# YuvalBahat/Explorable-Super-Resolution

Hardware: AMD Instinct MI355X
Metric: HR pixels/sec (RRDB-23 x4, 128->512, bs32 per GPU, fwd + CEM) (higher is better)
Workload: dtype bf16x3 (bf16 hi+lo operands = 16 significand bits per operand in every product, three MFMAs, f32 accumulate)

## Files before the change

### explorable-super-resolution_amd/csrc/esr_conv.hip

```cpp
#include "esr_common.h"
#include <type_traits>
#include <vector>

namespace {

constexpr int NW = 4;
constexpr int NTHREADS = 64 * NW;
constexpr int MAXS_BASE = 3;
constexpr int WGS_MT1 = 2, WGS_MT2 = 2;
constexpr int r_of(int mt) { return 3; }
constexpr int maxs_of(int mt) { return r_of(mt) > 3 ? MAXS_BASE + 1 : MAXS_BASE; }

typedef __attribute__((ext_vector_type(4))) unsigned int u32x4;
constexpr int EPI_RES1 = 1, EPI_RES2 = 2, EPI_MASK = 4, EPI_NCHW = 8, EPI_OUT2 = 16;
constexpr int EPI_RESIN = 32;
constexpr int EPI_PS = 64;

struct ConvArgs {
    int tiles_x, tiles_y, ntiles;
    int xcd_q, xcd_r;
    unsigned m_tx, m_ty;
    unsigned i_tx, i_ty;
    int TH, TW, P, NPIX_T, NPIX_L, nslots;
    unsigned m_P, m_ups;
    int H, W, Win_p, ups;
    unsigned share[NW];
    int ncp, lo_chunks, reverse, B;
    DView in0, in1;
    const uint4* wpack;
    long long wchunk;
    long long wslice;
    int wtap;
    int nslices;
    const float* zero_bias;
    int bias_stride;
    const float* bias;
    int cout, ncg_out;
    float act_slope, alpha, beta1, beta2;
    DView res1, res2, out, out2, mask;
    float* out_nchw;
    int mask_cg0, mask_cg1;
    float mask_slope;
    int resin_g0;
    float resin_scale;
    int ps, ps_rg0;
    unsigned m_ns, i_ns;
    int ph_off;
    int ksplit, kz_groups;
    long long kz_slab;
    int nchw_ctot;
    int stages_hint;
    unsigned* range_flag;
    unsigned range_tag;
#ifdef ESR_TRACE
    unsigned long long* trace;
#endif
};

typedef __attribute__((ext_vector_type(8))) _Float16 f16x8;
typedef __attribute__((ext_vector_type(2))) float f32x2;
template <int FMT>
__device__ __forceinline__ f32x16 mfma(uint4 a, uint4 b, f32x16 c) {
    if (FMT) return __builtin_amdgcn_mfma_f32_32x32x16_f16(__builtin_bit_cast(f16x8, a), __builtin_bit_cast(f16x8, b), c, 0, 0, 0);
    return __builtin_amdgcn_mfma_f32_32x32x16_bf16(__builtin_bit_cast(bf16x8, a), __builtin_bit_cast(bf16x8, b), c, 0, 0, 0);
}
template <int FMT>
__device__ __forceinline__ uint32_t cvt_pk(float lo, float hi);

__device__ __forceinline__ uint32_t cvt_pk_bf16(float lo, float hi) {
    uint32_t r;
    asm("v_cvt_pk_bf16_f32 %0, %1, %2" : "=v"(r) : "v"(lo), "v"(hi));
    return r;
}
template <> __device__ __forceinline__ uint32_t cvt_pk<0>(float lo, float hi) { return cvt_pk_bf16(lo, hi); }
template <> __device__ __forceinline__ uint32_t cvt_pk<1>(float lo, float hi) { return f2h(lo) | (f2h(hi) << 16); }

__device__ __forceinline__ void glds16s(const uint4* sbase, unsigned voff, unsigned lds_dst) {
    asm volatile("s_mov_b32 m0, %2\n\ts_nop 0\n\tglobal_load_lds_dwordx4 %0, %1" : : "v"(voff), "s"(sbase), "s"(__builtin_amdgcn_readfirstlane(lds_dst)) : "memory");
}

__device__ __forceinline__ unsigned udiv_magic(unsigned n, unsigned m, unsigned i) { return __umulhi(n, m) + n * i; }

__device__ __forceinline__ const uint4* in_plane(const ConvArgs& a, int g, int b, bool lo) {
    if (g < a.in0.ncg) return (lo ? a.in0.lo : a.in0.hi) + b * a.in0.bs + g * a.in0.cs;
    int g1 = g - a.in0.ncg;
    if (g1 >= a.in1.ncg) g1 = 0;
    return (lo ? a.in1.lo : a.in1.hi) + b * a.in1.bs + g1 * a.in1.cs;
}

template <int MAXS>
struct FetchState {
    unsigned soff[MAXS];
    int slot[MAXS];
};

template <int MAXS>
__device__ __forceinline__ FetchState<MAXS> setup_tile(const ConvArgs& a, int x0, int y0, int wave, int lane) {
    FetchState<MAXS> f;
#pragma unroll
    for (int s = 0; s < MAXS; ++s) {
        f.slot[s] = (wave + s * NW) < a.nslots ? wave + s * NW : wave;
        const unsigned p = (unsigned)f.slot[s] * 64 + lane;
        const unsigned rr = __umul24(p, a.m_P) >> 20, cc = p - rr * a.P;
        const unsigned Yp = y0 + rr, Xp = x0 + cc;
        const bool inb = (p < (unsigned)a.NPIX_T) && (Yp < (unsigned)a.H + 2) && (Xp < (unsigned)a.W + 2);
        const unsigned sy = __umul24(Yp + a.ups - 1, a.m_ups) >> 16, sx = __umul24(Xp + a.ups - 1, a.m_ups) >> 16;
        f.soff[s] = p >= (unsigned)a.NPIX_L ? ~0u : (inb ? (sy * a.Win_p + sx) * 16 : 0);
    }
    return f;
}

template <int NPL>
struct Bases {
    const uint4* p[2 * NPL];
    const uint4* w;
    int wtap;
};
template <int NPL, int MT, int NPW>
__device__ __forceinline__ Bases<NPL> make_bases(const ConvArgs& a, int cp, int b) {
    Bases<NPL> r;
#pragma unroll
    for (int i = 0; i < 2 * NPL; ++i) r.p[i] = in_plane(a, 2 * cp + i / NPL, b, (i % NPL) == 1);
    r.w = a.wpack + (size_t)cp * a.wchunk;
    r.wtap = a.wtap;
    return r;
}

struct DmaShare {
    int nsl;
    int w0, wc;
};
__device__ __forceinline__ DmaShare unpack_share(unsigned w) { return DmaShare{(int)(w & 0xFF), (int)((w >> 8) & 0xFF), (int)(w >> 16)}; }
template <int NPL, int MT = 1, int NPW = 1, int TMODE = 0>
__device__ __forceinline__ int dma_count(const DmaShare& d, bool xlo) { return (xlo ? 2 * NPL : 2) * d.nsl + (TMODE != 0 ? MT * NPW : d.wc); }

template <int NPL, int MT, int NPW, int TMODE = 0>
__device__ __forceinline__ void dma_chunk(const FetchState<maxs_of(MT)>& f, const Bases<NPL>& bs, const DmaShare& d, unsigned stage, int plane_bytes, bool xlo,
                                          int tsel = 0, int wave = 0) {
    constexpr int MAXS = maxs_of(MT);
#pragma unroll
    for (int s = 0; s < MAXS; ++s) {
        if (s >= d.nsl) break;
        const unsigned dst = stage + (unsigned)f.slot[s] * 1024;
        if (f.soff[s] != ~0u) {
#pragma unroll
            for (int cgpl = 0; cgpl < 2 * NPL; ++cgpl) {
                if (!xlo && (cgpl % NPL) == 1) continue;
                glds16s(bs.p[cgpl], f.soff[s], dst + cgpl * plane_bytes);
            }
        }
    }
    const unsigned vlane = (unsigned)(threadIdx.x & 63) * 16;
    if constexpr (TMODE == 0 && MT == 1) {
        for (int j = d.w0; j < d.w0 + d.wc; ++j) glds16s(bs.w + ((j / NPW) * bs.wtap + j % NPW) * 64, vlane, stage + 2 * NPL * plane_bytes + j * 1024);
    } else if constexpr (TMODE == 0) {
        for (int j = d.w0; j < d.w0 + d.wc; ++j) glds16s(bs.w + j * 64, vlane, stage + 2 * NPL * plane_bytes + j * 1024);
    } else {
        static_assert(TMODE == 0 || NW == 4, "one live tap per wave");
#pragma unroll
        for (int m = 0; m < MT; ++m) {
            const int r0 = TMODE == 1 ? 1 - (tsel >> 1) : tsel, c0 = TMODE == 1 ? 1 - (tsel & 1) : m;
            const int tap = (r0 + (wave >> 1)) * 3 + c0 + (wave & 1);
#pragma unroll
            for (int pl = 0; pl < NPW; ++pl) {
                const int j = (tap * MT + m) * NPW + pl;
                glds16s(bs.w + j * 64, vlane, stage + 2 * NPL * plane_bytes + j * 1024);
            }
        }
    }
}

template <int MAXN>
__device__ __forceinline__ void wait_vm_upto(int n) {
#define ESR_VMC(k) case k: if constexpr (k <= MAXN) { asm volatile("s_waitcnt vmcnt(" #k ")" ::: "memory"); break; }
    switch (n) {
        ESR_VMC(1) ESR_VMC(2) ESR_VMC(3) ESR_VMC(4) ESR_VMC(5) ESR_VMC(6) ESR_VMC(7) ESR_VMC(8) ESR_VMC(9) ESR_VMC(10) ESR_VMC(11) ESR_VMC(12)
        ESR_VMC(13) ESR_VMC(14) ESR_VMC(15) ESR_VMC(16) ESR_VMC(17) ESR_VMC(18) ESR_VMC(19) ESR_VMC(20) ESR_VMC(21) ESR_VMC(22) ESR_VMC(23)
        ESR_VMC(24) ESR_VMC(25) ESR_VMC(26) ESR_VMC(27) ESR_VMC(28) ESR_VMC(29) ESR_VMC(30) ESR_VMC(31) ESR_VMC(32)
        default: asm volatile("s_waitcnt vmcnt(0)" ::: "memory"); break;
    }
#undef ESR_VMC
}

struct ResRaw { uint4 h, l; };
__device__ __forceinline__ void swap_halves(const uint4& x, uint32_t (&d)[2][2]) {
    const auto s0 = __builtin_amdgcn_permlane32_swap(x.x, x.z, false, false);
    const auto s1 = __builtin_amdgcn_permlane32_swap(x.y, x.w, false, false);
    d[0][0] = s0[0]; d[0][1] = s1[0]; d[1][0] = s0[1]; d[1][1] = s1[1];
}
template <int FMT>
__device__ __forceinline__ void res_unpack(const ResRaw& q, bool has_lo, f32x2 (&rv)[2][2]) {
    uint32_t d[2][2];
    swap_halves(q.h, d);
#pragma unroll
    for (int k = 0; k < 2; ++k)
#pragma unroll
        for (int j = 0; j < 2; ++j) rv[k][j] = f32x2{e2f<FMT>(d[k][j] & 0xFFFF), e2f<FMT>(d[k][j] >> 16)};
    if (has_lo) {
        swap_halves(q.l, d);
#pragma unroll
        for (int k = 0; k < 2; ++k)
#pragma unroll
            for (int j = 0; j < 2; ++j) rv[k][j] += f32x2{e2f<FMT>(d[k][j] & 0xFFFF), e2f<FMT>(d[k][j] >> 16)};
    }
}

template <int NPL, int MT, int R, int FMT>
__device__ __forceinline__ void resin_accumulate(f32x16 (&acc)[MT][R], const ConvArgs& a, const unsigned char* stage, int cp, bool xlo, int P,
                                                 int plane_bytes, int wave, int lane) {
#pragma unroll
    for (int sgrp = 0; sgrp < 2; ++sgrp) {
        const int og = 2 * cp + sgrp - a.resin_g0;
        if (og < 0 || og * 8 >= a.cout) continue;
        float x[R][4];
#pragma unroll
        for (int r = 0; r < R; ++r) {
            const unsigned char* const pr = stage + sgrp * NPL * plane_bytes + ((wave + r * NW) * 32 + (lane & 31) + P + 1) * 16 + (lane >> 5) * 8;
            const uint2 h = *(const uint2*)pr;
            x[r][0] = e2f<FMT>(h.x & 0xFFFF); x[r][1] = e2f<FMT>(h.x >> 16); x[r][2] = e2f<FMT>(h.y & 0xFFFF); x[r][3] = e2f<FMT>(h.y >> 16);
            if (NPL == 2 && xlo) {
                const uint2 l = *(const uint2*)(pr + plane_bytes);
                x[r][0] += e2f<FMT>(l.x & 0xFFFF); x[r][1] += e2f<FMT>(l.x >> 16); x[r][2] += e2f<FMT>(l.y & 0xFFFF); x[r][3] += e2f<FMT>(l.y >> 16);
            }
        }
        auto add = [&](auto MG) {
            constexpr int mg = decltype(MG)::value;
            if constexpr (mg < MT * 4) {
#pragma unroll
                for (int r = 0; r < R; ++r)
#pragma unroll
                    for (int i = 0; i < 4; ++i) acc[mg / 4][r][(mg % 4) * 4 + i] = fmaf(a.resin_scale, x[r][i], acc[mg / 4][r][(mg % 4) * 4 + i]);
            }
        };
        switch (og) {
            case 0: add(std::integral_constant<int, 0>{}); break;
            case 1: add(std::integral_constant<int, 1>{}); break;
            case 2: add(std::integral_constant<int, 2>{}); break;
            case 3: add(std::integral_constant<int, 3>{}); break;
            case 4: add(std::integral_constant<int, 4>{}); break;
            case 5: add(std::integral_constant<int, 5>{}); break;
            case 6: add(std::integral_constant<int, 6>{}); break;
            default: add(std::integral_constant<int, 7>{}); break;
        }
    }
}

template <int NPL, int MT, int R, int NPW, int FMT, bool XLO, int NTERM_CAP, int TM0 = 0x1FF, int TM1 = 0x1FF>
__device__ __forceinline__ void chunk_mfma(f32x16 (&acc)[MT][R], const unsigned char* sa, const unsigned char* sb, int P, int plane_bytes) {
    constexpr int TMU = TM0 | (MT == 2 ? TM1 : 0);
#define ESR_TAP_LIVE(t, m) ((((m) == 0 ? TM0 : TM1) >> (t)) & 1)
    constexpr int NPB = XLO ? NPL : 1;
    constexpr int NT_FULL = 1 + (NPW == 2 ? 1 : 0) + (NPB == 2 ? 1 : 0);
    constexpr int NTERM = NT_FULL < NTERM_CAP ? NT_FULL : NTERM_CAP;
    constexpr int NM = MT * R * NTERM;
    constexpr int NLA = MT * NPW, NLB = R * NPB, NL = NLA + NLB;
    constexpr int NSLOT = NM > NL ? NM : NL;
    uint4 fa[2][MT][NPW], fb[2][R][NPB];
    auto load_frag = [&](int t, int k, int buf) {
        const int tapoff = ((t / 3) * P + (t % 3)) * 16;
        if (!((TMU >> t) & 1)) return;
        if (k < MT) {
            const int pl = NPW == 2 ? 1 : 0;
            if (ESR_TAP_LIVE(t, k)) fa[buf][k][pl] = *(const uint4*)(sa + ((t * MT + k) * NPW + pl) * 1024);
        } else if (k < MT + R) {
            fb[buf][k - MT][0] = *(const uint4*)(sb + (k - MT) * NW * 512 + tapoff);
        } else if (NPW == 2 && k < 2 * MT + R) {
            const int idx = k - MT - R;
            if (ESR_TAP_LIVE(t, idx)) fa[buf][idx][0] = *(const uint4*)(sa + ((t * MT + idx) * NPW) * 1024);
        } else {
            const int idx = k - (NPW == 2 ? 2 * MT + R : MT + R);
            fb[buf][idx][NPB - 1] = *(const uint4*)(sb + idx * NW * 512 + tapoff + (NPB - 1) * plane_bytes);
        }
    };
#pragma unroll
    for (int k = 0; k < NL; ++k) load_frag(0, k, 0);
#pragma unroll
    for (int t = 0; t < 9; ++t) {
        const int cb = t & 1;
#pragma unroll
        for (int i = 0; i < NSLOT; ++i) {
            if (i < NM) {
                const int ti = i / (MT * R), rem = i % (MT * R), r = rem % R, m = rem / R;
                constexpr int has0 = NPW == 2 ? 1 : 0, has1 = NPB == 2 ? 1 : 0;
                const int skip = NT_FULL - NTERM;
                const int idx = ti + skip;
                const int term = (idx < has0) ? 0 : ((idx < has0 + has1) ? 1 : 2);
                const int pa = term == 0 ? 1 : 0, pb = term == 1 ? 1 : 0;
                if (!ESR_TAP_LIVE(t, m)) {
                } else acc[m][r] = mfma<FMT>(fa[cb][m][pa], fb[cb][r][pb], acc[m][r]);
            }
            if (t < 8 && i < NL) load_frag(t + 1, i, cb ^ 1);
            __builtin_amdgcn_sched_barrier(0);
        }
    }
}

#undef ESR_TAP_LIVE

constexpr int S2D_FWD[4] = {432, 216, 54, 27}, S2D_FLIP[4] = {27, 54, 216, 432};

template <int R>
struct EpiCoord {
    int lim[R];
    unsigned poff[R];
};
template <int R, int KIND>
__device__ __forceinline__ EpiCoord<R> epi_coords(const ConvArgs& a, int x0, int y0, int wave, int lane) {
    EpiCoord<R> e;
    const int half = lane >> 5;
#pragma unroll
    for (int r = 0; r < R; ++r) {
        const unsigned q = (wave + r * NW) * 32 + (lane & 31);
        const unsigned rr = __umul24(q, a.m_P) >> 20, cc = q - rr * a.P;
        const unsigned Y = y0 + rr, X = x0 + cc;
        const bool valid = (rr < (unsigned)a.TH) && (cc < (unsigned)a.TW) && (Y < (unsigned)a.H) && (X < (unsigned)a.W);
        e.lim[r] = valid ? (KIND == 1 ? a.ncg_out : a.ncg_out - half) : (KIND == 1 ? 0 : -1);
        if (KIND == 1) e.poff[r] = (__umul24(Y, a.W) + X) * 4;
        else if (KIND == 2) e.poff[r] = (Y << 16) | X;
        else if (KIND == 3) e.poff[r] = valid ? (__umul24(2 * Y + 1, 2 * a.W + 2) + 2 * X + 1) * 16 : 0;
        else e.poff[r] = valid ? (__umul24(Y + 1, a.W + 2) + X + 1) * 16 : 0;
    }
    return e;
}

template <int NPL, int MT, int R, int EPI, int FMT, bool PARTLO, bool PHASE = false>
__device__ __forceinline__ void conv_epilogue(const ConvArgs& a, f32x16 (&acc)[MT][R], const int b, const EpiCoord<R>& ec, const int lane) {
    constexpr bool HAS_R1 = (EPI & EPI_RES1) != 0, HAS_R2 = (EPI & EPI_RES2) != 0, HAS_MK = (EPI & EPI_MASK) != 0;
    constexpr bool NCHW = (EPI & EPI_NCHW) != 0, OUT2 = (EPI & EPI_OUT2) != 0, PS = (EPI & EPI_PS) != 0;
    const int half = lane >> 5;
    const long long bl = b;
    const f32x2 slope2 = {a.act_slope, a.act_slope}, alpha2 = {a.alpha, a.alpha};
    const char *r1h = nullptr, *r1l = nullptr, *r2h = nullptr, *r2l = nullptr, *mkh = nullptr;
    unsigned h1 = 0, h2 = 0, ho = 0, ho2 = 0;
    if constexpr (HAS_R1) {
        r1h = (const char*)(a.res1.hi + bl * a.res1.bs);
        r1l = a.res1.lo ? (const char*)(a.res1.lo + bl * a.res1.bs) : nullptr;
        h1 = half ? (unsigned)a.res1.cs * 16 : 0;
    }
    if constexpr (HAS_R2) {
        r2h = (const char*)(a.res2.hi + bl * a.res2.bs);
        r2l = a.res2.lo ? (const char*)(a.res2.lo + bl * a.res2.bs) : nullptr;
        h2 = half ? (unsigned)a.res2.cs * 16 : 0;
    }
    if constexpr (HAS_MK) {
        mkh = (const char*)(a.mask.hi + bl * a.mask.bs);
    }
    char *oh = nullptr, *ol = nullptr, *o2h = nullptr, *o2l = nullptr;
    if constexpr (!NCHW) {
        oh = (char*)(a.out.hi + bl * a.out.bs);
        ol = (NPL == 2 && a.out.lo) ? (char*)(a.out.lo + bl * a.out.bs) : nullptr;
        ho = half ? (unsigned)a.out.cs * 16 : 0;
        if constexpr (OUT2) {
            o2h = (char*)(a.out2.hi + bl * a.out2.bs);
            o2l = (NPL == 2 && a.out2.lo) ? (char*)(a.out2.lo + bl * a.out2.bs) : nullptr;
            ho2 = half ? (unsigned)a.out2.cs * 16 : 0;
        }
    }
    constexpr int OPREGS_R = MT * 2 * (((HAS_R1 ? 1 : 0) + (HAS_R2 ? 1 : 0)) * NPL + (HAS_MK ? 1 : 0)) * 4;
    constexpr bool ALL_FIRST = OPREGS_R * R <= 96;
    constexpr int RQ = ALL_FIRST ? R : 1;
    ResRaw q1[HAS_R1 ? RQ : 1][MT * 2], q2[HAS_R2 ? RQ : 1][MT * 2];
    uint4 qm[HAS_MK ? RQ : 1][MT * 2];
    unsigned big = 0;
    auto issue = [&](const int r) {
        const int rq = ALL_FIRST ? r : 0;
#pragma unroll
        for (int mp = 0; mp < MT * 2; ++mp) {
            const int cg0 = mp * 2;
            const bool ok = cg0 < ec.lim[r];
            if constexpr (HAS_R1) {
                const unsigned off = ok ? ec.poff[r] + h1 + cg0 * ((unsigned)a.res1.cs * 16) : 0;
                q1[rq][mp].h = *(const uint4*)(r1h + off);
                if (NPL == 2 && r1l) q1[rq][mp].l = *(const uint4*)(r1l + off);
            }
            if constexpr (HAS_R2) {
                const unsigned off = ok ? ec.poff[r] + h2 + cg0 * ((unsigned)a.res2.cs * 16) : 0;
                q2[rq][mp].h = *(const uint4*)(r2h + off);
                if (NPL == 2 && r2l) q2[rq][mp].l = *(const uint4*)(r2l + off);
            }
            if constexpr (HAS_MK) {
                const int cgm = cg0 + half - a.mask_cg0;
                const bool okm = ok && cgm >= 0 && cg0 + half < a.mask_cg1;
                const unsigned off = okm ? ec.poff[r] + (unsigned)cgm * ((unsigned)a.mask.cs * 16) : 0;
                qm[rq][mp] = *(const uint4*)(mkh + off);
            }
        }
    };
    if constexpr (ALL_FIRST && (HAS_R1 || HAS_R2 || HAS_MK)) {
#pragma unroll
        for (int r = 0; r < R; ++r) issue(r);
    }
#pragma unroll
    for (int r = 0; r < R; ++r) {
        if constexpr (!ALL_FIRST && (HAS_R1 || HAS_R2 || HAS_MK)) issue(r);
        const int rq = ALL_FIRST ? r : 0;
#pragma unroll
        for (int m = 0; m < MT; ++m) {
#pragma unroll
            for (int gp = 0; gp < 2; ++gp) {
                const int cg0 = (PHASE ? 0 : m * 4) + gp * 2;
                if (!(cg0 < ec.lim[r] + (NCHW ? 0 : half))) continue;
                const bool store = cg0 < ec.lim[r];
                f32x2 v[2][2];
#pragma unroll
                for (int k = 0; k < 2; ++k)
#pragma unroll
                    for (int j = 0; j < 2; ++j) {
                        v[k][j] = f32x2{acc[m][r][(gp * 2 + k) * 4 + 2 * j], acc[m][r][(gp * 2 + k) * 4 + 2 * j + 1]} * alpha2;
                        v[k][j] = __builtin_elementwise_max(v[k][j], v[k][j] * slope2);
                    }
                if constexpr (HAS_R1) {
                    f32x2 rv[2][2];
                    res_unpack<FMT>(q1[rq][m * 2 + gp], NPL == 2 && a.res1.lo != nullptr, rv);
                    const f32x2 bb = {a.beta1, a.beta1};
#pragma unroll
                    for (int k = 0; k < 2; ++k)
#pragma unroll
                        for (int j = 0; j < 2; ++j) v[k][j] = __builtin_elementwise_fma(bb, rv[k][j], v[k][j]);
                }
                if constexpr (HAS_R2) {
                    f32x2 rv[2][2];
                    res_unpack<FMT>(q2[rq][m * 2 + gp], NPL == 2 && a.res2.lo != nullptr, rv);
                    const f32x2 bb = {a.beta2, a.beta2};
#pragma unroll
                    for (int k = 0; k < 2; ++k)
#pragma unroll
                        for (int j = 0; j < 2; ++j) v[k][j] = __builtin_elementwise_fma(bb, rv[k][j], v[k][j]);
                }
                if constexpr (HAS_MK) {
                    uint32_t d[2][2];
                    swap_halves(qm[rq][m * 2 + gp], d);
#pragma unroll
                    for (int k = 0; k < 2; ++k) {
                        const int cg = cg0 + k;
                        const float ms = (cg < a.mask_cg0 || cg >= a.mask_cg1) ? 1.f : a.mask_slope;
#pragma unroll
                        for (int j = 0; j < 2; ++j) {
                            const f32x2 s = v[k][j] * f32x2{ms, ms};
                            v[k][j].x = (int)(d[k][j] << 16) > 0 ? v[k][j].x : s.x;
                            v[k][j].y = (int)d[k][j] > 0xFFFF ? v[k][j].y : s.y;
                        }
                    }
                }
                if constexpr (NCHW) {
                    char* const ob = (char*)(a.out_nchw + bl * a.nchw_ctot * a.H * a.W);
                    const unsigned hw4 = (unsigned)(a.H * a.W) * 4;
#pragma unroll
                    for (int k = 0; k < 2; ++k) {
                        const int ch0 = (cg0 + k) * 8 + half * 4;
#pragma unroll
                        for (int i = 0; i < 4; ++i)
                            if (ch0 + i < a.cout) *(float*)(ob + (ec.poff[r] + (unsigned)(ch0 + i) * hw4)) = v[k][i >> 1][i & 1];
                    }
                    continue;
                }
                uint32_t hi[2][2], lo[2][2];
#pragma unroll
                for (int k = 0; k < 2; ++k)
#pragma unroll
                    for (int j = 0; j < 2; ++j) {
                        const uint32_t h = cvt_pk<FMT>(v[k][j].x, v[k][j].y);
                        hi[k][j] = h;
                        if constexpr (FMT == 1) big |= (h & 0x7FFF7FFFu) + 0x08000800u;
                        lo[k][j] = 0;
                        if (NPL == 2) lo[k][j] = cvt_pk<FMT>(v[k][j].x - e2f<FMT>(h & 0xFFFF), v[k][j].y - e2f<FMT>(h >> 16));
                    }
                const auto s0 = __builtin_amdgcn_permlane32_swap(hi[0][0], hi[1][0], false, false);
                const auto s1 = __builtin_amdgcn_permlane32_swap(hi[0][1], hi[1][1], false, false);
                const uint4 hv = make_uint4(s0[0], s1[0], s0[1], s1[1]);
                uint4 lv = hv;
                if (NPL == 2) {
                    const auto t0 = __builtin_amdgcn_permlane32_swap(lo[0][0], lo[1][0], false, false);
                    const auto t1 = __builtin_amdgcn_permlane32_swap(lo[0][1], lo[1][1], false, false);
                    lv = make_uint4(t0[0], t1[0], t0[1], t1[1]);
                }
                unsigned off;
                if constexpr (PS) {
                    const int cgs = cg0 + half, rg = a.ps_rg0 + cgs, r2 = a.ps * a.ps, sp = rg % r2;
                    const int Y = ec.poff[r] >> 16, X = ec.poff[r] & 0xFFFF;
                    off = ((unsigned)(rg / r2) * (unsigned)a.out.cs + (unsigned)(a.ps * Y + sp / a.ps + 1) * (a.ps * a.W + 2) + (a.ps * X + sp % a.ps + 1)) * 16;
                } else off = ec.poff[r] + ho + cg0 * ((unsigned)a.out.cs * 16) + (PHASE ? (unsigned)a.ph_off + m * 16 : 0u);
                if (store) {
                    *(uint4*)(oh + off) = hv;
                    if (NPL == 2 && (!PARTLO || ol)) *(uint4*)(ol + off) = lv;
                    if constexpr (OUT2) {
                        const unsigned off2 = ec.poff[r] + ho2 + cg0 * ((unsigned)a.out2.cs * 16);
                        *(uint4*)(o2h + off2) = hv;
                        if (NPL == 2 && o2l) *(uint4*)(o2l + off2) = lv;
                    }
                }
            }
        }
    }
    if constexpr (FMT == 1 && !NCHW) {
        if (a.range_flag && (big & 0x80008000u)) atomicMin(a.range_flag, a.range_tag);
    }
}

template <int MT>
__device__ __forceinline__ void bias_seed(const float* bias, int half, float (&bz)[MT][16]) {
    typedef const __attribute__((address_space(4))) float* cptr;
    const cptr cb = (cptr)(uintptr_t)bias;
#pragma unroll
    for (int m = 0; m < MT; ++m)
#pragma unroll
        for (int j = 0; j < 4; ++j)
#pragma unroll
            for (int k = 0; k < 4; ++k) {
                const int c0 = (m * 4 + j) * 8;
                const float lo = cb[c0 + k], hi = cb[c0 + 4 + k];
                bz[m][j * 4 + k] = half ? hi : lo;
            }
}

template <int NPL, int MT, int EPI, int NST, int FMT, int NPW, bool PARTLO, int TMODE = 0>
__global__ __launch_bounds__(NTHREADS, NST >= 2 ? 1 : (MT == 1 ? WGS_MT1 : WGS_MT2)) void conv3x3_tile_kernel(const ConvArgs a_in) {
    ConvArgs a = a_in;
    unsigned slice = blockIdx.y, tile3 = 0;
    if constexpr (TMODE == 3) {
        static_assert(TMODE != 3 || (MT == 2 && EPI == 0), "the phase launch: two phases per workgroup, plain epilogue");
        const unsigned xcd3 = blockIdx.x & 7;
        unsigned wg = xcd3 * a.xcd_q + (xcd3 < (unsigned)a.xcd_r ? xcd3 : (unsigned)a.xcd_r) + (blockIdx.x >> 3);
        if (a.reverse) wg = (unsigned)a.ntiles * a.nslices - 1 - wg;
        tile3 = udiv_magic(wg, a.m_ns, a.i_ns);
        slice = wg - tile3 * a.nslices;
        const long long blk = slice >> 1;
        a.wpack += (long long)slice * a.wslice;
        a.bias += blk * 32 * a.bias_stride;
        a.out.hi += blk * 4 * a.out.cs;
        if (a.out.lo) a.out.lo += blk * 4 * a.out.cs;
        a.ncg_out = a.ncg_out - 4 * (int)blk < 4 ? a.ncg_out - 4 * (int)blk : 4;
        a.ph_off = (slice & 1) ? (2 * a.W + 2) * 16 : 0;
    } else {
        const long long sl = blockIdx.y;
        a.wpack += sl * a.wslice;
        a.bias += sl * (MT * 32) * a.bias_stride;
        auto shift = [&](DView& v) { if (v.hi) { v.hi += sl * (MT * 4) * v.cs; if (v.lo) v.lo += sl * (MT * 4) * v.cs; } };
        shift(a.out); shift(a.out2); shift(a.res1); shift(a.res2);
        a.mask_cg0 -= (int)sl * (MT * 4);
        a.mask_cg1 -= (int)sl * (MT * 4);
        if constexpr ((EPI & EPI_RESIN) != 0) a.resin_g0 += (int)sl * (MT * 4);
        if constexpr ((EPI & EPI_NCHW) != 0) {
            a.out_nchw += sl * (MT * 32) * (long long)a.H * a.W;
            if (a.ksplit > 1) {
                const long long kz = blockIdx.z;
                a.in1.hi += kz * a.kz_groups * a.in1.cs;
                if (a.in1.lo) a.in1.lo += kz * a.kz_groups * a.in1.cs;
                a.wpack += kz * a.ncp * (9 * MT * NPW * 64);
                a.out_nchw += kz * a.kz_slab;
                if (kz) a.bias = a.zero_bias;
            }
        }
    }
    static_assert(!PARTLO || NPL == 2, "partial lo needs hi+lo activations");
    static_assert(NPW <= NPL, "a lo weight plane needs hi+lo activations");
    constexpr int R = r_of(MT), MAXS = maxs_of(MT);
    extern __shared__ __attribute__((aligned(16))) unsigned char smem[];
    const int tid = threadIdx.x;
    const int lane = tid & 63;
    const int wave = __builtin_amdgcn_readfirstlane(tid >> 6);
    const int P = a.P;
    const int plane_bytes = a.NPIX_L * 16;
    constexpr int NWI = 9 * MT * NPW;
    constexpr int MAXCNT = 2 * NPL * MAXS + (NWI + NW - 1) / NW;
    const int stage_bytes = 2 * NPL * plane_bytes + NWI * 1024;
    const unsigned xcd = blockIdx.x & 7;
    const unsigned tile_f = xcd * a.xcd_q + (xcd < (unsigned)a.xcd_r ? xcd : (unsigned)a.xcd_r) + (blockIdx.x >> 3);
    const unsigned tile = TMODE == 3 ? tile3 : (a.reverse ? a.ntiles - 1 - tile_f : tile_f);
    const unsigned trow = udiv_magic(tile, a.m_tx, a.i_tx);
    const int b = udiv_magic(trow, a.m_ty, a.i_ty);
    const int x0 = (tile - trow * a.tiles_x) * a.TW, y0 = (trow - b * a.tiles_y) * a.TH;
    const DmaShare share = unpack_share(a_in.share[wave]);
    const unsigned lds0 = (unsigned)(size_t)(__attribute__((address_space(3))) unsigned char*)smem;
#ifdef ESR_TRACE
    unsigned long long* const tr = a.trace ? a.trace + (size_t)blockIdx.x * 128 : nullptr;
    int tslot = 2;
    if (tr && tid == 0) { tr[0] = __builtin_amdgcn_s_getreg((31 << 11) | 4); tr[1] = __builtin_amdgcn_s_getreg((31 << 11) | 20); tr[126] = wall_clock64(); }
#define ESR_TR() do { if (tr && tid == 0 && tslot < 126) tr[tslot++] = __builtin_readcyclecounter(); } while (0)
    ESR_TR();
#else
#define ESR_TR() do { } while (0)
#endif
    const FetchState<MAXS> fs = setup_tile<MAXS>(a, x0, y0, wave, lane);
    ESR_TR();
    static_assert((TMODE != 2 && TMODE != 3) || MT == 2, "M-tile tap masks come in pairs");
    const unsigned char* const sb0 = smem + (lane >> 5) * NPL * plane_bytes + (wave * 32 + (lane & 31)) * 16;
    const unsigned char* const sa0 = smem + 2 * NPL * plane_bytes + lane * 16;
    constexpr int NTERM_CAP = 3;
    auto tsel_of = [&](const int c) { return TMODE == 1 ? ((c >> 1) & 3) : (TMODE == 2 || TMODE == 3 ? (int)(slice & 1) : 0); };
    auto issue = [&](const int c, const unsigned stage, const bool xlo) {
        const Bases<NPL> bs = make_bases<NPL, MT, NPW>(a, c, b);
        dma_chunk<NPL, MT, NPW, TMODE>(fs, bs, share, stage, plane_bytes, xlo, tsel_of(c), wave);
    };
    if (NST == 4) {
        static_assert(NST != 4 || !PARTLO, "the four-stage ring counts its copies per chunk: one count for all chunks");
#pragma unroll
        for (int c = 0; c < 3; ++c)
            if (c < a.ncp) issue(c, lds0 + c * stage_bytes, true);
    }
    constexpr int EKIND = TMODE == 3 ? 3 : ((EPI & EPI_NCHW) ? 1 : ((EPI & EPI_PS) ? 2 : 0));
    constexpr bool EARLY_COORDS = NST >= 2 || (MT == 1 && NPL == 1);
    f32x16 acc[MT][R];
    EpiCoord<R> ec;
    auto seed = [&]() {
        int lane_o = lane;
        asm volatile("" : "+v"(lane_o));
        constexpr int MB = TMODE == 3 ? 1 : MT;
        float bz[MB][16];
        bias_seed<MB>(a.bias, lane_o >> 5, bz);
#pragma unroll
        for (int m = 0; m < MT; ++m)
#pragma unroll
            for (int r = 0; r < R; ++r)
#pragma unroll
                for (int i = 0; i < 16; ++i) acc[m][r][i] = bz[m % MB][i];
        if constexpr (EARLY_COORDS) ec = epi_coords<R, EKIND>(a, x0, y0, wave, lane_o);
    };
    if (NST != 4) issue(0, lds0, !PARTLO || 0 < a.lo_chunks);
    __builtin_amdgcn_sched_barrier(0);
    ESR_TR();
    seed();
    ESR_TR();
    auto step = [&](auto XLO_T, const int cp) {
        constexpr bool xlo = decltype(XLO_T)::value;
        const int st = NST == 4 ? (cp & 3) : (NST >= 2 ? (cp & 1) : 0);
        const unsigned char* const sb = sb0 + st * stage_bytes;
        const unsigned char* const sa = sa0 + st * stage_bytes;
        ESR_TR();
        if (NST == 1) {
            if (cp > 0) issue(cp, lds0, xlo);
            ESR_TR();
            asm volatile("s_waitcnt vmcnt(0)" ::: "memory");
        } else if (NST == 4) {
            if (cp + 3 < a.ncp) issue(cp + 3, lds0 + ((cp + 3) & 3) * stage_bytes, true);
            const int ahead = a.ncp - 1 - cp < 3 ? a.ncp - 1 - cp : 3;
            ESR_TR();
            wait_vm_upto<3 * MAXCNT < 32 ? 3 * MAXCNT : 32>(ahead * dma_count<NPL, MT, NPW, TMODE>(share, true));
        } else {
            const bool more = cp + 1 < a.ncp;
            const bool xlo_next = !PARTLO || cp + 1 < a.lo_chunks;
            if (more) issue(cp + 1, lds0 + ((cp + 1) & 1) * stage_bytes, xlo_next);
            ESR_TR();
            wait_vm_upto<MAXCNT>(more ? dma_count<NPL, MT, NPW, TMODE>(share, xlo_next) : 0);
        }
        ESR_TR();
        __syncthreads();
        ESR_TR();
        if constexpr (TMODE == 1) {
            switch ((cp >> 1) & 3) {
                case 0: chunk_mfma<NPL, MT, R, NPW, FMT, xlo, NTERM_CAP, S2D_FWD[0], S2D_FWD[0]>(acc, sa, sb, P, plane_bytes); break;
                case 1: chunk_mfma<NPL, MT, R, NPW, FMT, xlo, NTERM_CAP, S2D_FWD[1], S2D_FWD[1]>(acc, sa, sb, P, plane_bytes); break;
                case 2: chunk_mfma<NPL, MT, R, NPW, FMT, xlo, NTERM_CAP, S2D_FWD[2], S2D_FWD[2]>(acc, sa, sb, P, plane_bytes); break;
                default: chunk_mfma<NPL, MT, R, NPW, FMT, xlo, NTERM_CAP, S2D_FWD[3], S2D_FWD[3]>(acc, sa, sb, P, plane_bytes); break;
            }
        } else if constexpr (TMODE == 2) {
            if (blockIdx.y & 1) chunk_mfma<NPL, MT, R, NPW, FMT, xlo, NTERM_CAP, S2D_FLIP[2], S2D_FLIP[3]>(acc, sa, sb, P, plane_bytes);
            else chunk_mfma<NPL, MT, R, NPW, FMT, xlo, NTERM_CAP, S2D_FLIP[0], S2D_FLIP[1]>(acc, sa, sb, P, plane_bytes);
        } else if constexpr (TMODE == 3) {
            const int py = slice & 1;
            chunk_mfma<NPL, MT, R, NPW, FMT, xlo, NTERM_CAP, S2D_FLIP[0], S2D_FLIP[1]>(acc, sa + py * (3 * MT * NPW * 1024), sb + py * (P * 16), P, plane_bytes);
        } else {
            chunk_mfma<NPL, MT, R, NPW, FMT, xlo, NTERM_CAP>(acc, sa, sb, P, plane_bytes);
        }
        if constexpr ((EPI & EPI_RESIN) != 0) resin_accumulate<NPL, MT, R, FMT>(acc, a, smem + st * stage_bytes, cp, xlo, P, plane_bytes, wave, lane);
        ESR_TR();
        __syncthreads();
    };
    const int lo_end = PARTLO ? (a.lo_chunks < a.ncp ? a.lo_chunks : a.ncp) : a.ncp;
    for (int cp = 0; cp < lo_end; ++cp) step(std::true_type{}, cp);
    if constexpr (PARTLO)
        for (int cp = lo_end; cp < a.ncp; ++cp) step(std::false_type{}, cp);
    ESR_TR();
    if constexpr (!EARLY_COORDS) ec = epi_coords<R, EKIND>(a, x0, y0, wave, lane);
    conv_epilogue<NPL, MT, R, EPI, FMT, PARTLO, TMODE == 3>(a, acc, b, ec, lane);
    ESR_TR();
#ifdef ESR_TRACE
    if (tr && tid == 0) tr[127] = wall_clock64();
#endif
}

__device__ __forceinline__ float fold2_tap(const float* w9, int t, int phase) {
    const int py = phase >> 1, px = phase & 1, ty = t / 3, tx = t % 3;
    if (ty < py || ty > py + 1 || tx < px || tx > px + 1) return 0.f;
    const int r0 = ty == py ? 0 : py + 1, r1 = ty == py ? py : 2;
    const int c0 = tx == px ? 0 : px + 1, c1 = tx == px ? px : 2;
    float a = w9[r0 * 3 + c0];
    if (r1 != r0) a = __fadd_rn(a, w9[r1 * 3 + c0]);
    if (c1 != c0) {
        float b = w9[r0 * 3 + c1];
        if (r1 != r0) b = __fadd_rn(b, w9[r1 * 3 + c1]);
        a = __fadd_rn(a, b);
    }
    return a;
}
__global__ void pack_weights_kernel(const float* __restrict__ w, int dim0, int dim1, const int* __restrict__ kmap, int ncg_in,
                                    const int* __restrict__ mmap, int mtiles, int transposed, int npl, int f16, float scale, uint4* __restrict__ out, int total) {
    const int idx = blockIdx.x * blockDim.x + threadIdx.x;
    if (idx >= total) return;
    const int lane = idx & 63;
    const int m = (idx >> 6) % mtiles;
    const int ks = (idx >> 6) / mtiles;
    const int cp = ks / 9, t = ks % 9;
    const int cg = 2 * cp + (lane >> 5);
    const int mch = mmap[m * 32 + (lane & 31)];
    float v8[8];
#pragma unroll
    for (int e = 0; e < 8; ++e) {
        const int kch = cg < ncg_in ? kmap[cg * 8 + e] : -1;
        float v = 0.f;
        if (kch >= 0 && mch >= 0) {
            if (transposed >= 2) v = fold2_tap(w + ((long long)mch * dim1 + kch) * 9, t, (transposed - 2 + m) & 3);
            else v = transposed ? w[((long long)kch * dim1 + mch) * 9 + (8 - t)] : w[((long long)mch * dim1 + kch) * 9 + t];
        }
        v8[e] = v * scale;
    }
    uint4* o = out + ((size_t)(ks * mtiles + m) * npl) * 64 + lane;
    store8(o, npl == 2 ? o + 64 : nullptr, 0, v8, f16 ? ESR_FMT_F16 : ESR_FMT_BF16);
}

struct PackEntry {
    const float* w; const int* kmap; const int* mmap; uint4* out;
    int dim0, dim1, ncg_in, mtiles, transposed, npl, f16, total; float scale;
};
__global__ __launch_bounds__(256) void pack_weights_batch_kernel(const PackEntry* __restrict__ table, const int2* __restrict__ map) {
    constexpr int PITCH = 16 * 9 + 1;
    __shared__ float tile[32 * PITCH];
    __shared__ int kch_s[16], mch_s[32];
    const int2 m = map[blockIdx.x];
    const PackEntry e = table[m.x];
    const int cp = m.y / e.mtiles, mt = m.y % e.mtiles;
    if (threadIdx.x < 16) {
        const int cg = 2 * cp + (threadIdx.x >> 3);
        kch_s[threadIdx.x] = cg < e.ncg_in ? e.kmap[cg * 8 + (threadIdx.x & 7)] : -1;
    } else if (threadIdx.x >= 32 && threadIdx.x < 64) mch_s[threadIdx.x - 32] = e.mmap[mt * 32 + (threadIdx.x - 32)];
    __syncthreads();
#pragma unroll
    for (int j = 0; j < 18; ++j) {
        const int f = j * 256 + threadIdx.x;
        int mr, kc, t;
        if (e.transposed == 1) { kc = f / 288; const int c = f - kc * 288; mr = c / 9; t = 8 - (c - mr * 9); }
        else { mr = f / 144; const int c = f - mr * 144; kc = c / 9; t = c - kc * 9; }
        const int kch = kch_s[kc], mch = mch_s[mr];
        float v = 0.f;
        if (kch >= 0 && mch >= 0) v = e.transposed == 1 ? e.w[((long long)kch * e.dim1 + mch) * 9 + (8 - t)] : e.w[((long long)mch * e.dim1 + kch) * 9 + t];
        tile[mr * PITCH + kc * 9 + t] = v;
    }
    __syncthreads();
    for (int v = threadIdx.x; v < 9 * 64; v += 256) {
        const int t = v >> 6, lane = v & 63;
        const float* src = tile + (lane & 31) * PITCH + (lane >> 5) * 72 + t;
        float x8[8];
#pragma unroll
        for (int c = 0; c < 8; ++c) x8[c] = (e.transposed >= 2 ? fold2_tap(src + c * 9 - t, t, (e.transposed - 2 + mt) & 3) : src[c * 9]) * e.scale;
        uint4* o = e.out + ((size_t)((cp * 9 + t) * e.mtiles + mt) * e.npl) * 64 + lane;
        store8(o, e.npl == 2 ? o + 64 : nullptr, 0, x8, e.f16 ? ESR_FMT_F16 : ESR_FMT_BF16);
    }
}

struct TileCfg { int TH, TW, P, NPIX_T, NPIX_L, tiles_x, tiles_y; size_t lds; };
constexpr size_t stage_bytes(int npl, int npix_l, int mt, int npw) { return (size_t)2 * npl * npix_l * 16 + (size_t)9 * mt * npw * 1024; }

TileCfg pick_tile_search(int H, int W, int npl, int mt, int nwg);
TileCfg pick_tile(int H, int W, int npl, int mt, int nwg) {
    struct Entry { int H, W, npl, mt, nwg; TileCfg cfg; };
    static thread_local Entry cache[8];
    static thread_local int next = 0;
    for (const Entry& e : cache)
        if (e.H == H && e.W == W && e.npl == npl && e.mt == mt && e.nwg == nwg && e.cfg.P) return e.cfg;
    Entry& e = cache[next];
    next = (next + 1) % 8;
    e = Entry{H, W, npl, mt, nwg, pick_tile_search(H, W, npl, mt, nwg)};
    return e.cfg;
}
TileCfg pick_tile_search(int H, int W, int npl, int mt, int nwg) {
    const int R = r_of(mt), MAXS = maxs_of(mt);
    TileCfg best{};
    double best_cost = -1;
    const size_t budget = 160 * 1024;
    const int max_px = 32 * NW * R;
    for (int ntx = 1; ntx <= W; ++ntx) {
        const int TW = (W + ntx - 1) / ntx;
        const int P = TW + 2;
        if (P > max_px) continue;
        if (ntx > 1 && TW < 6) break;
        int THmax = max_px / P;
        if (THmax > H) THmax = H;
        for (int TH = THmax; TH >= 1 && TH >= THmax - 6; --TH) {
            const int npix_t = (TH + 2) * P;
            int npix_l = max_px + 2 * P + 2;
            if (npix_l < npix_t) npix_l = npix_t;
            if (npix_l > MAXS * NW * 64) continue;
            const size_t lds = nwg * stage_bytes(npl, npix_l, mt, npl);
            if (lds > budget) continue;
            const int nty = (H + TH - 1) / TH;
            const double halo = (double)(TH + 2) * P / ((double)TH * TW);
            const double cost = (double)ntx * nty * (1.0 + 0.05 * halo);
            if (best_cost < 0 || cost < best_cost) {
                best_cost = cost;
                best = TileCfg{TH, TW, P, npix_t, npix_l, ntx, nty, lds};
            }
        }
    }
    return best;
}

#ifdef ESR_TRACE
unsigned long long* g_trace = nullptr;
#endif

__device__ float g_zero_bias[64];
const float* zero_bias() {
    static const float* ptr[64] = {};
    int dev = 0;
    (void)hipGetDevice(&dev);
    const float*& p = ptr[dev & 63];
    if (!p) {
        void* q = nullptr;
        if (hipGetSymbolAddress(&q, HIP_SYMBOL(g_zero_bias)) != hipSuccess) return nullptr;
        p = (const float*)q;
    }
    return p;
}

void dma_share_host(int npl, int nwi, int nslots, unsigned (&out)[NW]) {
    const int target = (2 * npl * nslots + nwi + NW - 1) / NW;
    int start = 0;
    for (int v = 0; v < NW; ++v) {
        const int nv = nslots > v ? (nslots - v + NW - 1) / NW : 0;
        int c = target - 2 * npl * nv;
        c = c < 0 ? 0 : c;
        if (c > nwi - start || v == NW - 1) c = nwi - start;
        out[v] = (unsigned)nv | ((unsigned)start << 8) | ((unsigned)c << 16);
        start += c;
    }
}

constexpr int CONV_SMALL_WGS = 320;

struct ConvPlan {
    bool phases, mslice;
    int npl, ps, nslices, mt;
    int mt_k, kslices;
    TileCfg tile;
    int ups, fmt, wpl;
    bool partlo;
    int in0g, ncp, lo_chunks;
    int tmode, epi, nst, S;
    int resin_g0;
    float resin_scale;
    dim3 grid;
    size_t lds;
};

template <int... V> struct Ints {};
template <int... V> constexpr bool among(Ints<V...>, int v) { return ((v == V) || ...); }

typedef Ints<0, EPI_RES1, EPI_RES1 | EPI_RES2, EPI_RESIN, EPI_RESIN | EPI_RES2, EPI_NCHW, EPI_OUT2, EPI_RES1 | EPI_MASK, EPI_MASK, EPI_PS> ConvEpis;
constexpr bool has_ring4(int mt, int epi, int fmt, bool partlo, int tmode) { return (epi == 0 || epi == EPI_NCHW) && !partlo && fmt == 0 && mt == 2 && tmode != 3; }
constexpr bool two_stages_only(int npl, int tmode) { return (tmode == 1 || tmode == 2) && npl == 2; }

constexpr bool conv_kernel_exists(int npl, int mt, int epi, int nst, int fmt, int npw, bool partlo, int tmode) {
    if (fmt == 0 ? (npw != npl || partlo) : (npw > npl || (partlo && npl == 1))) return false;
    if (nst == 4 ? !has_ring4(mt, epi, fmt, partlo, tmode) : (nst == 1 && two_stages_only(npl, tmode))) return false;
    if (tmode == 0) return among(ConvEpis{}, epi);
    if (mt != 2 || partlo) return false;
    return tmode == 3 ? epi == 0 : (fmt == 0 && (epi == 0 || epi == EPI_NCHW));
}

typedef void (*ConvKernel)(const ConvArgs);
template <int NPL, int MT, int EPI, int NST, int FMT, int NPW, int PARTLO, int TMODE>
ConvKernel conv_pick(Ints<NPL, MT, EPI, NST, FMT, NPW, PARTLO, TMODE>, const int*) {
    if constexpr (conv_kernel_exists(NPL, MT, EPI, NST, FMT, NPW, PARTLO != 0, TMODE)) {
        ConvKernel k = conv3x3_tile_kernel<NPL, MT, EPI, NST, FMT, NPW, PARTLO != 0, TMODE>;
        ESR_ALLOW_160K_LDS(k);
        return k;
    } else return nullptr;
}
template <int... C, int... V, class... More>
ConvKernel conv_pick(Ints<C...>, const int* v, Ints<V...>, More... more) {
    ConvKernel k = nullptr;
    ((*v == V ? void(k = conv_pick(Ints<C..., V>{}, v + 1, more...)) : void()), ...);
    return k;
}
ConvKernel conv_kernel(const ConvPlan& p) {
    const int v[8] = {p.npl, p.mt_k, p.epi, p.nst, p.fmt, p.wpl, p.partlo, p.tmode};
    return conv_pick(Ints<>{}, v, Ints<1, 2>{}, Ints<1, 2>{}, ConvEpis{}, Ints<1, 2, 4>{}, Ints<0, 1>{}, Ints<1, 2>{}, Ints<0, 1>{}, Ints<0, 1, 2, 3>{});
}

__global__ void splitk_finish_kernel(const float* __restrict__ ws, int S, long long slab, DView out, int C, int H, int W, long long total) {
    const long long idx = (long long)blockIdx.x * blockDim.x + threadIdx.x;
    if (idx >= total) return;
    const ActPos q = act_pos(idx, C >> 3, H, W);
    const int b = q.b, cg = q.cg, y = q.y, x = q.x;
    float v8[8];
#pragma unroll
    for (int e = 0; e < 8; ++e) {
        const float* p = ws + ((long long)(b * C + cg * 8 + e) * H + y) * W + x;
        float v = 0.f;
        for (int k = 0; k < S; ++k) v += p[k * slab];
        v8[e] = v;
    }
    store8(mut(out.hi), mut(out.lo), act_off(out.bs, out.cs, W, b, cg, y, x), v8, ESR_FMT_BF16);
}

}

#ifdef ESR_TRACE
extern "C" void esr_debug_trace(void* buf) { g_trace = (unsigned long long*)buf; }
#endif

extern "C" size_t esr_conv_wpack_bytes(int ncg_in, int cout, int split) {
    const int ncp = (ncg_in + 1) / 2, mt = (cout + 31) / 32;
    return (size_t)ncp * 9 * mt * ((split == 1 || split == 3) ? 2 : 1) * 64 * 16;
}

extern "C" int esr_pack_conv_weights(const float* w, int cout_w, int cin_w, const int32_t* kmap, int ncg_in, const int32_t* mmap,
                                     int mtiles, int transposed, int split, float scale, void* wpack, esr_stream_t stream) {
    if (!w || !kmap || !mmap || !wpack || ncg_in <= 0 || mtiles <= 0 || transposed < 0 || transposed > 5) return ESR_E_ARG;
    const int ncp = (ncg_in + 1) / 2;
    const int total = ncp * 9 * mtiles * 64;
    ESR_CLEAR_ERR();
    hipLaunchKernelGGL(pack_weights_kernel, dim3((total + 255) / 256), dim3(256), 0, (hipStream_t)stream, w, cout_w, cin_w, kmap,
                       ncg_in, mmap, mtiles, transposed, (split == 1 || split == 3) ? 2 : 1, split >= 2 ? 1 : 0, scale, (uint4*)wpack, total);
    ESR_CHECK_LAUNCH();
    return ESR_OK;
}

static int64_t pack_batch_blocks(const esr_pack_desc* descs, int n) {
    int64_t nb = 0;
    for (int i = 0; i < n; ++i) {
        if (!descs[i].w || !descs[i].kmap || !descs[i].mmap || !descs[i].wpack || descs[i].ncg_in <= 0 || descs[i].mtiles <= 0 || descs[i].transposed < 0 ||
            descs[i].transposed > 5)
            return ESR_E_ARG;
        nb += (int64_t)((descs[i].ncg_in + 1) / 2) * descs[i].mtiles;
    }
    return nb;
}

extern "C" int64_t esr_pack_batch_workspace_bytes(const esr_pack_desc* descs, int n) {
    if (!descs || n <= 0) return ESR_E_ARG;
    const int64_t nb = pack_batch_blocks(descs, n);
    if (nb < 0) return nb;
    return ((int64_t)n * sizeof(PackEntry) + 255) / 256 * 256 + nb * (int64_t)sizeof(int2);
}

extern "C" int64_t esr_pack_batch_upload(const esr_pack_desc* descs, int n, void* workspace, int64_t workspace_bytes, esr_stream_t stream) {
    if (!descs || n <= 0 || !workspace) return ESR_E_ARG;
    const int64_t need = esr_pack_batch_workspace_bytes(descs, n);
    if (need < 0 || workspace_bytes < need) return ESR_E_ARG;
    const int64_t nb = pack_batch_blocks(descs, n);
    std::vector<PackEntry> table(n);
    std::vector<int2> map((size_t)nb);
    int64_t b = 0;
    for (int i = 0; i < n; ++i) {
        PackEntry& e = table[i];
        e.w = descs[i].w; e.kmap = descs[i].kmap; e.mmap = descs[i].mmap; e.out = (uint4*)descs[i].wpack;
        e.dim0 = descs[i].cout_w; e.dim1 = descs[i].cin_w; e.ncg_in = descs[i].ncg_in; e.mtiles = descs[i].mtiles;
        e.transposed = descs[i].transposed; e.npl = (descs[i].split == 1 || descs[i].split == 3) ? 2 : 1; e.f16 = descs[i].split >= 2 ? 1 : 0; e.scale = descs[i].scale;
        e.total = ((descs[i].ncg_in + 1) / 2) * 9 * descs[i].mtiles * 64;
        for (int j = 0; j < ((descs[i].ncg_in + 1) / 2) * descs[i].mtiles; ++j) map[(size_t)b++] = make_int2(i, j);
    }
    const size_t tb = ((size_t)n * sizeof(PackEntry) + 255) / 256 * 256;
    hipStream_t s = (hipStream_t)stream;
    if (hipMemcpyAsync(workspace, table.data(), (size_t)n * sizeof(PackEntry), hipMemcpyHostToDevice, s) != hipSuccess) return ESR_E_LAUNCH;
    if (hipMemcpyAsync((char*)workspace + tb, map.data(), (size_t)nb * sizeof(int2), hipMemcpyHostToDevice, s) != hipSuccess) return ESR_E_LAUNCH;
    return nb;
}

extern "C" int esr_pack_batch_run(const void* workspace, int n, int64_t nblocks, esr_stream_t stream) {
    if (!workspace || n <= 0 || nblocks <= 0) return ESR_E_ARG;
    const size_t tb = ((size_t)n * sizeof(PackEntry) + 255) / 256 * 256;
    ESR_CLEAR_ERR();
    hipLaunchKernelGGL(pack_weights_batch_kernel, dim3((unsigned)nblocks), dim3(256), 0, (hipStream_t)stream, (const PackEntry*)workspace,
                       (const int2*)((const char*)workspace + tb));
// ... 216 lines not shown
```

Before: 127.7 million.

## Split residual-input chunk loop into plain and compile-time residual spans

For kernels with a fused residual input, the channel-chunk loop is split into chunks before, inside and after the range that carries residual groups. Plain chunks skip the per-chunk residual check and runtime switch entirely. In the single-stage pipeline, residual chunks are unrolled with compile-time group indices so the FMA targets fixed accumulator registers. The cost is more code and instruction-cache pressure from the extra unrolled step copies.

Result: faster. 129.5 million, median of 6 (+1.5%).

```diff
diff --git a/explorable-super-resolution_amd/csrc/esr_conv.hip b/explorable-super-resolution_amd/csrc/esr_conv.hip
--- a/explorable-super-resolution_amd/csrc/esr_conv.hip
+++ b/explorable-super-resolution_amd/csrc/esr_conv.hip
@@ -15,6 +15,7 @@
 constexpr int EPI_RES1 = 1, EPI_RES2 = 2, EPI_MASK = 4, EPI_NCHW = 8, EPI_OUT2 = 16;
 constexpr int EPI_RESIN = 32;
 constexpr int EPI_PS = 64;
+constexpr int RES_PLAIN = -2, RES_LOOP = -1;
 
 struct ConvArgs {
     int tiles_x, tiles_y, ntiles;
@@ -205,6 +206,28 @@
     }
 }
 
+template <int NPL, int R, int FMT>
+__device__ __forceinline__ void resin_load(float (&x)[R][4], const unsigned char* stage, int sgrp, bool xlo, int P, int plane_bytes, int wave, int lane) {
+#pragma unroll
+    for (int r = 0; r < R; ++r) {
+        const unsigned char* const pr = stage + sgrp * NPL * plane_bytes + ((wave + r * NW) * 32 + (lane & 31) + P + 1) * 16 + (lane >> 5) * 8;
+        const uint2 h = *(const uint2*)pr;
+        x[r][0] = e2f<FMT>(h.x & 0xFFFF); x[r][1] = e2f<FMT>(h.x >> 16); x[r][2] = e2f<FMT>(h.y & 0xFFFF); x[r][3] = e2f<FMT>(h.y >> 16);
+        if (NPL == 2 && xlo) {
+            const uint2 l = *(const uint2*)(pr + plane_bytes);
+            x[r][0] += e2f<FMT>(l.x & 0xFFFF); x[r][1] += e2f<FMT>(l.x >> 16); x[r][2] += e2f<FMT>(l.y & 0xFFFF); x[r][3] += e2f<FMT>(l.y >> 16);
+        }
+    }
+}
+template <int MT, int R, int OG>
+__device__ __forceinline__ void resin_fma(f32x16 (&acc)[MT][R], float scale, const float (&x)[R][4]) {
+    if constexpr (OG >= 0 && OG < MT * 4) {
+#pragma unroll
+        for (int r = 0; r < R; ++r)
+#pragma unroll
+            for (int i = 0; i < 4; ++i) acc[OG / 4][r][(OG % 4) * 4 + i] = fmaf(scale, x[r][i], acc[OG / 4][r][(OG % 4) * 4 + i]);
+    }
+}
 template <int NPL, int MT, int R, int FMT>
 __device__ __forceinline__ void resin_accumulate(f32x16 (&acc)[MT][R], const ConvArgs& a, const unsigned char* stage, int cp, bool xlo, int P,
                                                  int plane_bytes, int wave, int lane) {
@@ -213,34 +236,34 @@
         const int og = 2 * cp + sgrp - a.resin_g0;
         if (og < 0 || og * 8 >= a.cout) continue;
         float x[R][4];
-#pragma unroll
-        for (int r = 0; r < R; ++r) {
-            const unsigned char* const pr = stage + sgrp * NPL * plane_bytes + ((wave + r * NW) * 32 + (lane & 31) + P + 1) * 16 + (lane >> 5) * 8;
-            const uint2 h = *(const uint2*)pr;
-            x[r][0] = e2f<FMT>(h.x & 0xFFFF); x[r][1] = e2f<FMT>(h.x >> 16); x[r][2] = e2f<FMT>(h.y & 0xFFFF); x[r][3] = e2f<FMT>(h.y >> 16);
-            if (NPL == 2 && xlo) {
-                const uint2 l = *(const uint2*)(pr + plane_bytes);
-                x[r][0] += e2f<FMT>(l.x & 0xFFFF); x[r][1] += e2f<FMT>(l.x >> 16); x[r][2] += e2f<FMT>(l.y & 0xFFFF); x[r][3] += e2f<FMT>(l.y >> 16);
-            }
-        }
-        auto add = [&](auto MG) {
-            constexpr int mg = decltype(MG)::value;
-            if constexpr (mg < MT * 4) {
-#pragma unroll
-                for (int r = 0; r < R; ++r)
-#pragma unroll
-                    for (int i = 0; i < 4; ++i) acc[mg / 4][r][(mg % 4) * 4 + i] = fmaf(a.resin_scale, x[r][i], acc[mg / 4][r][(mg % 4) * 4 + i]);
-            }
-        };
+        resin_load<NPL, R, FMT>(x, stage, sgrp, xlo, P, plane_bytes, wave, lane);
         switch (og) {
-            case 0: add(std::integral_constant<int, 0>{}); break;
-            case 1: add(std::integral_constant<int, 1>{}); break;
-            case 2: add(std::integral_constant<int, 2>{}); break;
-            case 3: add(std::integral_constant<int, 3>{}); break;
-            case 4: add(std::integral_constant<int, 4>{}); break;
-            case 5: add(std::integral_constant<int, 5>{}); break;
-            case 6: add(std::integral_constant<int, 6>{}); break;
-            default: add(std::integral_constant<int, 7>{}); break;
+            case 0: resin_fma<MT, R, 0>(acc, a.resin_scale, x); break;
+            case 1: resin_fma<MT, R, 1>(acc, a.resin_scale, x); break;
+            case 2: resin_fma<MT, R, 2>(acc, a.resin_scale, x); break;
+            case 3: resin_fma<MT, R, 3>(acc, a.resin_scale, x); break;
+            case 4: resin_fma<MT, R, 4>(acc, a.resin_scale, x); break;
+            case 5: resin_fma<MT, R, 5>(acc, a.resin_scale, x); break;
+            case 6: resin_fma<MT, R, 6>(acc, a.resin_scale, x); break;
+            default: resin_fma<MT, R, 7>(acc, a.resin_scale, x); break;
+        }
+    }
+}
+template <int NPL, int MT, int R, int FMT, int OG0>
+__device__ __forceinline__ void resin_accumulate_at(f32x16 (&acc)[MT][R], const ConvArgs& a, const unsigned char* stage, bool xlo, int P, int plane_bytes,
+                                                    int wave, int lane) {
+    if constexpr (OG0 >= 0 && OG0 < MT * 4) {
+        if (OG0 * 8 < a.cout) {
+            float x[R][4];
+            resin_load<NPL, R, FMT>(x, stage, 0, xlo, P, plane_bytes, wave, lane);
+            resin_fma<MT, R, OG0>(acc, a.resin_scale, x);
+        }
+    }
+    if constexpr (OG0 + 1 >= 0 && OG0 + 1 < MT * 4) {
+        if ((OG0 + 1) * 8 < a.cout) {
+            float x[R][4];
+            resin_load<NPL, R, FMT>(x, stage, 1, xlo, P, plane_bytes, wave, lane);
+            resin_fma<MT, R, OG0 + 1>(acc, a.resin_scale, x);
         }
     }
 }
@@ -621,7 +644,7 @@
     ESR_TR();
     seed();
     ESR_TR();
-    auto step = [&](auto XLO_T, const int cp) {
+    auto step = [&](auto XLO_T, auto RES_T, const int cp) __attribute__((always_inline)) {
         constexpr bool xlo = decltype(XLO_T)::value;
         const int st = NST == 4 ? (cp & 3) : (NST >= 2 ? (cp & 1) : 0);
         const unsigned char* const sb = sb0 + st * stage_bytes;
@@ -662,14 +685,53 @@
         } else {
             chunk_mfma<NPL, MT, R, NPW, FMT, xlo, NTERM_CAP>(acc, sa, sb, P, plane_bytes);
         }
-        if constexpr ((EPI & EPI_RESIN) != 0) resin_accumulate<NPL, MT, R, FMT>(acc, a, smem + st * stage_bytes, cp, xlo, P, plane_bytes, wave, lane);
+        if constexpr (decltype(RES_T)::value == RES_LOOP) {
+            resin_accumulate<NPL, MT, R, FMT>(acc, a, smem + st * stage_bytes, cp, xlo, P, plane_bytes, wave, lane);
+        } else if constexpr (decltype(RES_T)::value >= 0) {
+            constexpr int k = decltype(RES_T)::value;
+            if (a.resin_g0 & 1) {
+                asm volatile("; residual chunk, odd first group");
+                resin_accumulate_at<NPL, MT, R, FMT, 2 * k - 1>(acc, a, smem + st * stage_bytes, xlo, P, plane_bytes, wave, lane);
+                asm volatile("; residual chunk, odd first group: end");
+            } else {
+                asm volatile("; residual chunk, even first group");
+                resin_accumulate_at<NPL, MT, R, FMT, 2 * k>(acc, a, smem + st * stage_bytes, xlo, P, plane_bytes, wave, lane);
+                asm volatile("; residual chunk, even first group: end");
+            }
+        }
         ESR_TR();
         __syncthreads();
     };
+    constexpr std::integral_constant<int, RES_PLAIN> PLAIN{};
+    auto span = [&](auto XLO_T, const int c0, const int c1) {
+        if constexpr ((EPI & EPI_RESIN) != 0) {
+            const int rc0 = a.resin_g0 >> 1, rc1 = (a.resin_g0 + ((a.cout + 7) >> 3) + 1) >> 1;
+            const int r0 = rc0 < c0 ? c0 : (rc0 > c1 ? c1 : rc0), r1 = rc1 < r0 ? r0 : (rc1 > c1 ? c1 : rc1);
+            for (int cp = c0; cp < r0; ++cp) step(XLO_T, PLAIN, cp);
+            if constexpr (NST == 1) {
+                auto res_chunk = [&](auto KC) __attribute__((always_inline)) {
+                    if constexpr (decltype(KC)::value < MT * 2 + 1) {
+                        const int cp = rc0 + decltype(KC)::value;
+                        if (cp >= r0 && cp < r1) step(XLO_T, KC, cp);
+                    }
+                };
+                res_chunk(std::integral_constant<int, 0>{}); res_chunk(std::integral_constant<int, 1>{}); res_chunk(std::integral_constant<int, 2>{});
+                res_chunk(std::integral_constant<int, 3>{}); res_chunk(std::integral_constant<int, 4>{});
+            } else {
+                for (int cp = r0; cp < r1; ++cp) step(XLO_T, std::integral_constant<int, RES_LOOP>{}, cp);
+            }
+            for (int cp = r1; cp < c1; ++cp) step(XLO_T, PLAIN, cp);
+        }
+    };
     const int lo_end = PARTLO ? (a.lo_chunks < a.ncp ? a.lo_chunks : a.ncp) : a.ncp;
-    for (int cp = 0; cp < lo_end; ++cp) step(std::true_type{}, cp);
-    if constexpr (PARTLO)
-        for (int cp = lo_end; cp < a.ncp; ++cp) step(std::false_type{}, cp);
+    if constexpr ((EPI & EPI_RESIN) != 0) {
+        span(std::true_type{}, 0, lo_end);
+        if constexpr (PARTLO) span(std::false_type{}, lo_end, a.ncp);
+    } else {
+        for (int cp = 0; cp < lo_end; ++cp) step(std::true_type{}, PLAIN, cp);
+        if constexpr (PARTLO)
+            for (int cp = lo_end; cp < a.ncp; ++cp) step(std::false_type{}, PLAIN, cp);
+    }
     ESR_TR();
     if constexpr (!EARLY_COORDS) ec = epi_coords<R, EKIND>(a, x0, y0, wave, lane);
     conv_epilogue<NPL, MT, R, EPI, FMT, PARTLO, TMODE == 3>(a, acc, b, ec, lane);
```
